# Saltfish-AB/LatentSync

Hardware: AMD Instinct MI355X
Metric: lip-synced frames/sec at 256x256, 16-frame window, 20 DDIM steps (higher is better)
Workload: dtype bf16; 1 GPU; configs[1]: 256x256 x16-frame windows, 20 DDIM steps, guidance 1.0, LatentSync-1.5 UNet + SD-VAE, bf16; 48 independent windows of a clip batched per UNet call; windows_per_rank=240, windows_per_batch=48, frames_per_window=16, global_batch=768, resolution=256, parallelism=dp1 (window sharding, RCCL all-gather of decoded frames)

## Files before the change

### latentsync_amd/csrc/ls_ff.hip

```cpp
#include "ls_common.h"

namespace ls {

struct FFArgs {
  const u16* x;
  const float* ln_mr;
  const u16* w1;
  const float* b1;
  const u16* w2;
  const float* b2;
  u16* y;
  long M;
  int ldx, ldy;
};

template <int C, int I, int PD1 = 2, int PD2 = 6>
__global__ void __launch_bounds__(512, 1) ff_fused_kernel(FFArgs a) {
  constexpr int KT = C / 32;
  constexpr int NCH = I / 32;
  constexpr int WIMG = 64 * (C / 64) * 8;
  constexpr int W2IMG = C * 4;
  constexpr int STAGE = WIMG + W2IMG;
  constexpr int NT2 = C / 16;
  constexpr int PW1 = WIMG / 512;
// ... 107 lines not shown
#pragma unroll
    for (int t = 0; t < NT2; ++t) {
      const int col = 16 * t + 4 * lg;
      const float4 b = *(const float4*)(a.b2 + col);
      const uint2 rs = *(const uint2*)(xr + col);
      const float o0 = out[t][0] + b.x + __uint_as_float(rs.x << 16);
      const float o1 = out[t][1] + b.y + __uint_as_float(rs.x & 0xffff0000u);
      const float o2 = out[t][2] + b.z + __uint_as_float(rs.y << 16);
      const float o3 = out[t][3] + b.w + __uint_as_float(rs.y & 0xffff0000u);
      *(uint2*)(yr + col) = make_uint2(pack2(o0, o1), pack2(o2, o3));
    }
  }
}

struct FFChainArgs {
  const u16* o;
  const u16* wo;
  const float* bo;
  const u16* h1;
  const u16* w1;
  const float* b1;
  const u16* w2;
  const float* b2;
  const u16* wp;
  const float* bp;
  const u16* xb;
  u16* z;
  float* cs_out;
  long M;
  int ldo, ldh, ldxb, ldz;
  float eps;
};

template <int C, int I>
__global__ void __launch_bounds__(512, 1) ff_chain_kernel(FFChainArgs a) {
  constexpr int FMR = 1;
  constexpr int NW = 8 / FMR;
  constexpr int NT = 64 * NW;
  constexpr int KT = C / 32;
  constexpr int NCH = I / 32;
  constexpr int WIMG = 64 * (C / 64) * 8;
  constexpr int W2IMG = C * 4;
  constexpr int STAGE = WIMG + W2IMG;
  constexpr int KPS = STAGE / W2IMG;
  constexpr int NA = (KT + KPS - 1) / KPS;
  constexpr int NT2 = C / 16;
  constexpr int PW1 = WIMG / NT;
  constexpr int UW2 = W2IMG / 64;
  constexpr int PD1 = 2, PD2 = 6;
  constexpr int ZP = C + 8;
  constexpr int RG = NT >= C ? 4 : 2;
  static_assert(STAGE % W2IMG == 0 && KPS >= 1 && WIMG % NT == 0, "ff_chain stage layout");
  static_assert(2 * STAGE * 16 >= 128 * ZP * 2 + RG * (C / 4) * 8 * 4, "ff_chain epilogue LDS");
  static_assert(C == 320 && I == 1280, "ff_chain shape");
  extern __shared__ __attribute__((aligned(16))) uint4 lds[];
  float* b1s = (float*)(lds + 2 * STAGE);

  const int tid = threadIdx.x, lane = tid & 63, wid = tid >> 6;
  const int l16 = lane & 15, lg = lane >> 4;
  const long row0 = (long)blockIdx.x * 128;
  const int wr0 = wid * 16 * FMR + l16;

  for (int i = tid; i < 2 * I / 4; i += NT) ((float4*)b1s)[i] = ((const float4*)a.b1)[i];

  const int wid_u = __builtin_amdgcn_readfirstlane(wid);
  __builtin_assume(wid_u >= 0 && wid_u < NW);
  const i32x4 rs_w1 = buffer_rsrc(a.w1, (uint32_t)(2L * I * C * 2));
  const i32x4 rs_w2 = buffer_rsrc(a.w2, (uint32_t)((long)I * C * 2));
  const i32x4 rs_wo = buffer_rsrc(a.wo, (uint32_t)((long)C * C * 2));
  const i32x4 rs_wp = buffer_rsrc(a.wp, (uint32_t)((long)C * C * 2));
  int vo1[PW1];
#pragma unroll
  for (int p = 0; p < PW1; ++p) {
    const int q = p * NT + tid, r = (q >> 3) & 63, pc = q & 7;
    const int lc = pc ^ ((r >> 1) & 7);
    vo1[p] = (r * C + (q >> 9) * 64 + lc * 8) * 2;
  }
  const int vol = (wid_u * 64 + lane) * 16;
  lds_u4* const lbase = (lds_u4*)lds;
  auto issue = [&](int g, int st) __attribute__((always_inline)) {
    lds_u4* const dst = lbase + st * STAGE;
    if (g < NA || g >= NA + NCH) {
      const bool o = g < NA;
      const int q = o ? g : g - NA - NCH;
      const int nk = min(KPS, KT - q * KPS);
      const int so = q * KPS * W2IMG * 16;
      for (int k = 0; wid_u + k * NW < nk * UW2; ++k)
        ls_raw_buffer_load_lds(o ? rs_wo : rs_wp, (__attribute__((address_space(3))) void*)(dst + (wid_u + k * NW) * 64),
                               16, vol + k * NW * 1024, so, 0, 0);
    } else {
      const int c = g - NA;
#pragma unroll
      for (int p = 0; p < PW1; ++p)
        ls_raw_buffer_load_lds(rs_w1, (__attribute__((address_space(3))) void*)(dst + p * NT + wid_u * 64), 16, vo1[p],
                               c * 64 * C * 2, 0, 0);
      for (int k = 0; wid_u + k * NW < UW2; ++k)
        ls_raw_buffer_load_lds(rs_w2, (__attribute__((address_space(3))) void*)(dst + WIMG + (wid_u + k * NW) * 64), 16,
                               vol + k * NW * 1024, c * W2IMG * 16, 0, 0);
    }
  };
  auto top = [&](int g) __attribute__((always_inline)) {
    wait_vm<0>();
    asm volatile("s_waitcnt lgkmcnt(0)" ::: "memory");
    __builtin_amdgcn_s_barrier();
    asm volatile("" ::: "memory");
    if (g + 1 < 2 * NA + NCH) issue(g + 1, (g + 1) & 1);
    return (const uint4*)(lds + (g & 1) * STAGE);
  };
  issue(0, 0);

  const int p2 = lg ^ (((l16 >> 3) & 1) << 1);
  bf16x8 ar[FMR][KT];
  f32x4 out[FMR][NT2];
  auto init_cols = [&](const float* v) __attribute__((always_inline)) {
#pragma unroll
    for (int t = 0; t < NT2; ++t) {
      const float4 b = *(const float4*)(v + 16 * t + 4 * lg);
#pragma unroll
      for (int f = 0; f < FMR; ++f) out[f][t] = (f32x4){b.x, b.y, b.z, b.w};
    }
  };
  auto proj = [&](int g0) __attribute__((always_inline)) {
#pragma unroll
    for (int q = 0; q < NA; ++q) {
      const uint4* cur = top(g0 + q);
      const int nk = (q + 1) * KPS <= KT ? KPS : KT - q * KPS;
      int lo[KPS];
#pragma unroll
      for (int j = 0; j < KPS; ++j) {
        lo[j] = j * W2IMG + l16 * 4 + p2;
        asm volatile("" : "+v"(lo[j]));
      }
      uint4 wq[PD2];
#pragma unroll
      for (int i = 0; i < PD2; ++i) wq[i] = cur[lo[i / NT2] + (i % NT2) * 64];
#pragma unroll
      for (int j = 0; j < KPS; ++j) {
        if (j < nk) {
          const int k = q * KPS + j < KT ? q * KPS + j : 0;
#pragma unroll
          for (int t = 0; t < NT2; ++t) {
            const int i = j * NT2 + t;
            const bf16x8 wv = __builtin_bit_cast(bf16x8, wq[i % PD2]);
            const int n = i + PD2;
            if (n < nk * NT2) wq[i % PD2] = cur[lo[n / NT2 < KPS ? n / NT2 : 0] + (n % NT2) * 64];
#pragma unroll
            for (int f = 0; f < FMR; ++f)
              out[f][t] = __builtin_amdgcn_mfma_f32_16x16x32_bf16(wv, ar[f][k], out[f][t], 0, 0, 0);
          }
          __builtin_amdgcn_sched_barrier(0);
        }
      }
    }
  };
  auto acc_to_operand = [&](int f, float mean, float rstd) __attribute__((always_inline)) {
#pragma unroll
    for (int s = 0; s < KT; ++s) {
      bf16x8 v;
#pragma unroll
      for (int e = 0; e < 8; ++e) v[e] = (__bf16)((out[f][2 * s + (e >> 2)][e & 3] - mean) * rstd);
      ar[f][s] = v;
    }
  };

#pragma unroll
  for (int f = 0; f < FMR; ++f) {
    const u16* src = a.o + (row0 + wr0 + 16 * f) * a.ldo + lg * 8;
#pragma unroll
    for (int s = 0; s < KT; ++s) ar[f][s] = *(const bf16x8*)(src + s * 32);
  }
  init_cols(a.bo);
  proj(0);
#pragma unroll
  for (int f = 0; f < FMR; ++f) {
    uint2 xr[NT2];
    const u16* hr = a.h1 + (row0 + wr0 + 16 * f) * a.ldh + 4 * lg;
#pragma unroll
    for (int t = 0; t < NT2; ++t) xr[t] = *(const uint2*)(hr + 16 * t);
    float s1 = 0.f;
#pragma unroll
    for (int t = 0; t < NT2; ++t) {
      const uint2 rs = xr[t];
      const uint32_t pk0 = pack2(out[f][t][0] + __uint_as_float(rs.x << 16), out[f][t][1] + __uint_as_float(rs.x & 0xffff0000u));
      const uint32_t pk1 = pack2(out[f][t][2] + __uint_as_float(rs.y << 16), out[f][t][3] + __uint_as_float(rs.y & 0xffff0000u));
      out[f][t] = (f32x4){__uint_as_float(pk0 << 16), __uint_as_float(pk0 & 0xffff0000u),
                          __uint_as_float(pk1 << 16), __uint_as_float(pk1 & 0xffff0000u)};
      s1 += (out[f][t][0] + out[f][t][1]) + (out[f][t][2] + out[f][t][3]);
    }
    const float mean = xor16_32_sum(s1) * (1.0f / C);
    float s2 = 0.f;
#pragma unroll
    for (int t = 0; t < NT2; ++t)
#pragma unroll
      for (int r = 0; r < 4; ++r) {
        const float d = out[f][t][r] - mean;
        s2 = fmaf(d, d, s2);
      }
    const float rstd = rsqrtf(xor16_32_sum(s2) * (1.0f / C) + a.eps);
    acc_to_operand(f, mean, rstd);
  }
#pragma unroll
  for (int t = 0; t < NT2; ++t) {
    const float4 b = *(const float4*)(a.b2 + 16 * t + 4 * lg);
#pragma unroll
    for (int f = 0; f < FMR; ++f) {
      out[f][t][0] += b.x; out[f][t][1] += b.y; out[f][t][2] += b.z; out[f][t][3] += b.w;
    }
  }

  for (int c = 0; c < NCH; ++c) {
    const uint4* cur = top(NA + c);
    f32x4 acc[FMR][4];
    const float* bb = b1s + c * 64 + 4 * lg;
#pragma unroll
    for (int f = 0; f < FMR; ++f)
#pragma unroll
      for (int t = 0; t < 4; ++t) acc[f][t] = (f32x4){0.f, 0.f, 0.f, 0.f};
    auto frag = [&](int s, int t) {
      return __builtin_bit_cast(bf16x8, cur[(s >> 1) * 512 + swz64(t * 16 + l16, (s & 1) * 4 + lg)]);
    };
    const uint4* w2 = cur + WIMG;
    bf16x8 wf[PD1][4];
#pragma unroll
    for (int p = 0; p < PD1; ++p)
#pragma unroll
      for (int t = 0; t < 4; ++t) wf[p][t] = frag(p, t);
    uint4 w2q[PD2];
#pragma unroll
    for (int s = 0; s < KT; ++s) {
      const int sl = s % PD1;
      bf16x8 cw[4];
#pragma unroll
      for (int t = 0; t < 4; ++t) cw[t] = wf[sl][t];
      if (s + PD1 < KT) {
#pragma unroll
        for (int t = 0; t < 4; ++t) wf[sl][t] = frag(s + PD1, t);
      } else if (s + PD1 - KT < PD2) {
        w2q[s + PD1 - KT] = w2[((s + PD1 - KT) * 16 + l16) * 4 + p2];
      }
#pragma unroll
      for (int t = 0; t < 4; ++t)
#pragma unroll
        for (int f = 0; f < FMR; ++f) acc[f][t] = __builtin_amdgcn_mfma_f32_16x16x32_bf16(cw[t], ar[f][s], acc[f][t], 0, 0, 0);
    }
#pragma unroll
    for (int q = PD1; q < PD2; ++q) w2q[q] = w2[(q * 16 + l16) * 4 + p2];
    bf16x8 gv[FMR];
#pragma unroll
    for (int f = 0; f < FMR; ++f)
#pragma unroll
      for (int r = 0; r < 4; ++r) {
        gv[f][r] = (__bf16)((acc[f][0][r] + bb[r]) * gelu_erf(acc[f][1][r] + bb[16 + r]));
        gv[f][4 + r] = (__bf16)((acc[f][2][r] + bb[32 + r]) * gelu_erf(acc[f][3][r] + bb[48 + r]));
      }
#pragma unroll
    for (int t = 0; t < NT2; ++t) {
      const bf16x8 wv = __builtin_bit_cast(bf16x8, w2q[t % PD2]);
      if (t + PD2 < NT2) w2q[t % PD2] = w2[((t + PD2) * 16 + l16) * 4 + p2];
#pragma unroll
      for (int f = 0; f < FMR; ++f) out[f][t] = __builtin_amdgcn_mfma_f32_16x16x32_bf16(wv, gv[f], out[f][t], 0, 0, 0);
    }
  }

#pragma unroll
  for (int f = 0; f < FMR; ++f) acc_to_operand(f, 0.f, 1.f);
  init_cols(a.bp);
  proj(NA + NCH);

  __syncthreads();
  u16* zimg = (u16*)lds;
#pragma unroll
  for (int f = 0; f < FMR; ++f) {
    uint2 xr[NT2];
    const u16* src = a.xb + (row0 + wr0 + 16 * f) * a.ldxb + 4 * lg;
#pragma unroll
    for (int t = 0; t < NT2; ++t) xr[t] = *(const uint2*)(src + 16 * t);
#pragma unroll
    for (int t = 0; t < NT2; ++t) {
      const uint2 rs = xr[t];
      const float o0 = out[f][t][0] + __uint_as_float(rs.x << 16), o1 = out[f][t][1] + __uint_as_float(rs.x & 0xffff0000u);
      const float o2 = out[f][t][2] + __uint_as_float(rs.y << 16), o3 = out[f][t][3] + __uint_as_float(rs.y & 0xffff0000u);
      *(uint2*)(zimg + (wr0 + 16 * f) * ZP + 16 * t + 4 * lg) = make_uint2(pack2(o0, o1), pack2(o2, o3));
    }
  }
  __syncthreads();
  constexpr int PCS = C / 8;
  for (int q = tid; q < 128 * PCS; q += NT) {
    const int r = q / PCS, ch = q - r * PCS;
    *(uint4*)(a.z + (row0 + r) * a.ldz + ch * 8) = *(const uint4*)(zimg + r * ZP + ch * 8);
  }
  if (a.cs_out) {
    constexpr int RPG = 128 / RG;
    float* part = (float*)(zimg + 128 * ZP);
    if (tid < RG * (C / 4)) {
      const int cq = tid % (C / 4), rg = tid / (C / 4);
      float s1[4] = {0.f, 0.f, 0.f, 0.f}, s2[4] = {0.f, 0.f, 0.f, 0.f};
      for (int r = 0; r < RPG; ++r) {
        const uint2 v = *(const uint2*)(zimg + (RPG * rg + r) * ZP + 4 * cq);
        const float fv[4] = {__uint_as_float(v.x << 16), __uint_as_float(v.x & 0xffff0000u),
                             __uint_as_float(v.y << 16), __uint_as_float(v.y & 0xffff0000u)};
// ... 14 lines not shown
        t2 += part[(rg * (C / 4) + cq) * 8 + 4 + e];
      }
      a.cs_out[(long)blockIdx.x * 2 * C + col] = t1;
      a.cs_out[(long)blockIdx.x * 2 * C + C + col] = t2;
    }
  }
}


}

using namespace ls;

extern "C" int ls_ff_chain(const ls_ff_chain_desc* d, void* stream) {
  if (!d || !d->o || !d->wo || !d->bo || !d->h1 || !d->w1 || !d->b1 || !d->w2 || !d->b2 || !d->wp || !d->bp ||
      !d->xb || !d->z)
    return fail(LS_ERR_INVALID, "ls_ff_chain: null pointer");
  if (d->C != 320 || d->inner != 1280) return fail(LS_ERR_INVALID, "ls_ff_chain: C = 320, inner = 1280 only");
  if (d->M <= 0 || d->M % 128 || (d->M / 128) > 0x7fffffffL)
    return fail(LS_ERR_INVALID, "ls_ff_chain: M a positive multiple of 128");
  if (d->ldo < d->C || d->ldh < d->C || d->ldxb < d->C || d->ldz < d->C || d->ldo % 8 || d->ldh % 4 ||
      d->ldxb % 4 || d->ldz % 8)
    return fail(LS_ERR_INVALID, "ls_ff_chain: pitches >= C (o, z: % 8; h1, xb: % 4)");
  if ((((uintptr_t)d->o | (uintptr_t)d->wo | (uintptr_t)d->w1 | (uintptr_t)d->w2 | (uintptr_t)d->wp |
        (uintptr_t)d->b1 | (uintptr_t)d->b2 | (uintptr_t)d->bo | (uintptr_t)d->bp | (uintptr_t)d->z |
        (uintptr_t)d->cs_out) & 15) || (((uintptr_t)d->h1 | (uintptr_t)d->xb) & 7))
    return fail(LS_ERR_INVALID, "ls_ff_chain: operands 16-B aligned (h1 / xb 8-B)");
  FFChainArgs a;
  a.o = (const u16*)d->o; a.wo = (const u16*)d->wo; a.bo = d->bo; a.h1 = (const u16*)d->h1;
  a.w1 = (const u16*)d->w1; a.b1 = d->b1; a.w2 = (const u16*)d->w2; a.b2 = d->b2;
  a.wp = (const u16*)d->wp; a.bp = d->bp; a.xb = (const u16*)d->xb; a.z = (u16*)d->z; a.cs_out = d->cs_out;
  a.M = d->M; a.ldo = d->ldo; a.ldh = d->ldh; a.ldxb = d->ldxb; a.ldz = d->ldz; a.eps = d->eps;
  constexpr int C = 320, I = 1280;
  const size_t shm = (size_t)2 * (64 * (C / 64) * 8 + C * 4) * 16 + 2 * I * sizeof(float);
  LS_SET_MAX_DYN_SHM((ff_chain_kernel<C, I>), (int)shm);
  ff_chain_kernel<C, I><<<(unsigned)(d->M / 128), 512, shm, (hipStream_t)stream>>>(a);
  return check_launch("ff_chain_kernel");
}

extern "C" int ls_feedforward(const ls_ff_desc* d, void* stream) {
  if (!d || !d->x || !d->ln_rowstats || !d->w1 || !d->b1 || !d->w2 || !d->b2 || !d->y)
    return fail(LS_ERR_INVALID, "ls_feedforward: null pointer");
  if (d->C != 320 || d->inner != 1280) return fail(LS_ERR_INVALID, "ls_feedforward: C = 320, inner = 1280 only");
  if (d->M <= 0 || d->ldx < d->C || d->ldy < d->C || d->ldx % 8 || d->ldy % 4)
    return fail(LS_ERR_INVALID, "ls_feedforward: bad rows / pitches (ldx % 8, ldy % 4, >= C)");
  if ((((uintptr_t)d->x | (uintptr_t)d->w1 | (uintptr_t)d->w2 | (uintptr_t)d->b1 | (uintptr_t)d->b2) & 15) ||
      (((uintptr_t)d->y | (uintptr_t)d->ln_rowstats) & 7))
    return fail(LS_ERR_INVALID, "ls_feedforward: x / w1 / w2 / b1 / b2 16-B aligned, y / ln_rowstats 8-B aligned");
  if ((d->M + 127) / 128 > 0x7fffffffL) return fail(LS_ERR_INVALID, "ls_feedforward: too many rows");
  FFArgs a;
  a.x = (const u16*)d->x; a.ln_mr = d->ln_rowstats; a.w1 = (const u16*)d->w1; a.b1 = d->b1;
  a.w2 = (const u16*)d->w2; a.b2 = d->b2; a.y = (u16*)d->y; a.M = d->M; a.ldx = d->ldx; a.ldy = d->ldy;
  constexpr int C = 320, I = 1280;
  const size_t shm = (size_t)2 * (64 * (C / 64) * 8 + C * 4) * 16 + 2 * I * sizeof(float);
  LS_SET_MAX_DYN_SHM((ff_fused_kernel<C, I>), (int)shm);
  ff_fused_kernel<C, I><<<(unsigned)((d->M + 127) / 128), 512, shm, (hipStream_t)stream>>>(a);
  return check_launch("ff_fused_kernel");
}
```

### latentsync_amd/ops.py

```python
import ctypes as C
import math

import torch

from . import _lib
from ._lib import check

ACT_NONE, ACT_GEGLU, ACT_GELU, ACT_SILU = 0, 1, 2, 3
_GN_EPILOGUE = True
GN_SLOT_ROWS = 128
_UPS_PHASE = True


def _p(t):
    return None if t is None else t.data_ptr()


def _stream():
    return torch.cuda.current_stream().cuda_stream


class Workspace:

    def __init__(self, device, gemm_bytes=256 << 20, gn_bytes=24 << 20):
# ... 278 lines not shown


def feedforward(x2d, ln_stats, w1: "Packed", w2: "Packed", w2ff, out=None):
    lib = _lib.load()
    M, C_ = x2d.shape
    if out is None:
        out = torch.empty((M, C_), dtype=torch.bfloat16, device=x2d.device)
    d = _lib.FFDesc()
    d.x, d.ln_rowstats, d.w1, d.b1 = _p(x2d), _p(ln_stats), _p(w1.w), _p(w1.bias)
    d.w2, d.b2, d.y = _p(w2ff), _p(w2.bias), _p(out)
    d.M, d.ldx, d.ldy, d.C, d.inner = M, x2d.stride(0), out.stride(0), C_, w1.N // 2
    check(lib.ls_feedforward(C.byref(d), _stream()), "ls_feedforward")
    return out


class FFChainPack:

    def __init__(self, wo, bo, w1, b1, w2, b2, wp, bp, C, inner, eps):
        self.wo, self.bo, self.w1, self.b1, self.w2, self.b2, self.wp, self.bp = wo, bo, w1, b1, w2, b2, wp, bp
        self.C, self.inner, self.eps = C, inner, eps


def pack_ff_chain(wo: "Packed", ff1: "Packed", ff2: "Packed", po: "Packed", eps=1e-5):
    from .packing import pack_ff_w2, permute_k_acc
    Cc = wo.N
    bf = lambda t: t.to(torch.bfloat16).contiguous()
    w1 = permute_k_acc(ff1.w.float())
    return FFChainPack(bf(pack_ff_w2(wo.w.float()[:, :Cc], permute=False)), wo.bias.float().contiguous(), bf(w1),
                       ff1.bias.float().contiguous(), bf(pack_ff_w2(ff2.w.float()[:, :ff2.K])),
                       ff2.bias.float().contiguous(), bf(pack_ff_w2(po.w.float()[:, :Cc])),
                       po.bias.float().contiguous(), Cc, ff1.N // 2, eps)


def ff_chain_ok(o2d, pk: "FFChainPack"):
    return (pk is not None and o2d.shape[1] == 320 and pk.inner == 1280 and o2d.shape[0] % 128 == 0
            and o2d.stride(1) == 1 and o2d.stride(0) % 8 == 0)


def ff_chain(o2d, h1, xb, pk: "FFChainPack", shape=None, gn_out=True):
    lib = _lib.load()
    M, C_ = o2d.shape
    res = torch.empty(shape or (M, C_), dtype=torch.bfloat16, device=o2d.device)
    out = res.view(M, C_)
    cs = torch.empty((M // GN_SLOT_ROWS, 2, C_), dtype=torch.float32, device=o2d.device) if gn_out else None
    d = _lib.FFChainDesc()
    d.o, d.wo, d.bo, d.h1 = _p(o2d), _p(pk.wo), _p(pk.bo), _p(h1)
    d.w1, d.b1, d.w2, d.b2, d.wp, d.bp = _p(pk.w1), _p(pk.b1), _p(pk.w2), _p(pk.b2), _p(pk.wp), _p(pk.bp)
    d.xb, d.z, d.cs_out = _p(xb), _p(out), _p(cs)
    d.M, d.ldo, d.ldh, d.ldxb, d.ldz = M, o2d.stride(0), h1.stride(0), xb.stride(0), out.stride(0)
    d.C, d.inner, d.eps = C_, pk.inner, float(pk.eps)
    check(lib.ls_ff_chain(C.byref(d), _stream()), "ls_ff_chain")
    if cs is not None:
        res.gn_cs = cs
    return res


class XAttnPack:

    def __init__(self, wq, bq, wo, bo, C, heads):
        self.wq, self.bq, self.wo, self.bo, self.C, self.heads = wq, bq, wo, bo, C, heads


def pack_cross_attention(wq, ln_weight, ln_bias, wo, bo, heads, device):
    from .packing import pack_xattn_q, pack_xattn_wo
    w = wq.float().cpu()
    gamma, beta = ln_weight.float().cpu(), ln_bias.float().cpu()
    pq, pb = pack_xattn_q(w * gamma[None, :], w @ beta, heads)
    po = pack_xattn_wo(wo.float().cpu(), heads)
    bf = lambda t: t.to(torch.bfloat16).to(device).contiguous()
# ... 442 lines not shown
```

### latentsync_amd/unet.py

```python
import math
from dataclasses import dataclass

import torch

from . import ops
from .config import STAGE2_MODEL
from .packing import geglu_interleave, pack_ff_w2, pack_phase_weight, pack_weight, pad_bias
from .schema import unet_param_shapes
from .weights import fill_state_dict

_FUSED_TEMPORAL = True
_FUSED_FF = True
_FF_CHAIN = True
_NARROW_OUT = True
_FUSED_XATTN = False


def _ff(h, st, ff1, ff2, ff2p):
    if ff2p is not None and ops.feedforward_ok(h, ff1, ff2):
        return ops.feedforward(h, st, ff1, ff2, ff2p)
    g = ops.linear(h, ff1, act=ops.ACT_GEGLU, ln_stats=st)
    return ops.linear(g, ff2, res=h)


# ... 139 lines not shown
        self.chain = _chain_pack(self.o2, self.ff1, self.ff2, self.proj_out, c) if self.has_audio else None

    def audio_kv(self, audio_rows):
        return ops.linear(audio_rows, self.kv2) if self.has_audio else None

    def __call__(self, x, audio_rows, n_audio_tok, kv=None):
        n, H, W, C = x.shape
        HW = H * W
        rows = n * HW
        d = C // self.heads
        sc = ops.group_norm(x, self.groups, 1e-6, *self.norm, n)
        st = torch.empty((rows, 2), dtype=torch.float32, device=x.device)
        h = ops.conv(x, self.proj_in, aff=(sc[0], sc[1], 1, False), aff_materialize=True,
                     stats_out=st).view(rows, C)
        qkv = ops.linear(h, self.qkv1, ln_stats=st)
        o = torch.empty((rows, C), dtype=torch.bfloat16, device=x.device)
        ops.attention(qkv, qkv[:, C:], qkv[:, 2 * C:], o, batch=n, z2=1, heads=self.heads, nq=HW, nk=HW, head_dim=d,
                      qs=(HW * 3 * C, 0, 3 * C, d), ks=(HW * 3 * C, 0, 3 * C, d), vs=(HW * 3 * C, 0, 3 * C, d),
                      os_=(HW * C, 0, C, d), fp8=self.fp8 and HW > 128 and d in (40, 80))
        h = ops.linear(o, self.o1, res=h, stats_out=st)
        if self.has_audio and audio_rows is not None:
            if kv is None:
                kv = ops.linear(audio_rows, self.kv2)
            L = n_audio_tok
            if ops.cross_attention_ok(h, self.xa, L, HW):
                st2 = torch.empty_like(st)
                h = ops.cross_attention_block(h, st, self.xa, kv, L, HW, st2)
                st = st2
                return self._tail(x, h, st, n, H, W, C)
            q = ops.linear(h, self.q2, ln_stats=st)
            ops.attention(q, kv, kv[:, C:], o, batch=n, z2=1, heads=self.heads, nq=HW, nk=L, head_dim=d,
                          qs=(HW * C, 0, C, d), ks=(L * 2 * C, 0, 2 * C, d), vs=(L * 2 * C, 0, 2 * C, d),
                          os_=(HW * C, 0, C, d))
            if ops.ff_chain_ok(o, self.chain):
                return ops.ff_chain(o, h, x.view(rows, C), self.chain, shape=(n, H, W, C))
            h = ops.linear(o, self.o2, res=h, stats_out=st)
        return self._tail(x, h, st, n, H, W, C)

    def _tail(self, x, h, st, n, H, W, C):
        h = _ff(h, st, self.ff1, self.ff2, self.ff2p)
        return ops.conv(h.view(n, H, W, C), self.proj_out, res=x, gn_out=True)


class _Motion:
    def __init__(self, dv, p, c, heads, groups, kw):
        t = p + ".temporal_transformer"
        b = t + ".transformer_blocks.0"
        sd = dv.sd
        self.c, self.heads, self.groups = c, heads, groups
        self.norm = (dv.f32(t + ".norm.weight"), dv.f32(t + ".norm.bias"))
        self.proj_in = dv.packed(t + ".proj_in.weight", t + ".proj_in.bias")
        self.proj_out = dv.packed(t + ".proj_out.weight", t + ".proj_out.bias")
        self.attn = []
        i = 0
        max_len = kw.get("temporal_position_encoding_max_len", 24)
        while f"{b}.attention_blocks.{i}.to_q.weight" in sd:
            a = f"{b}.attention_blocks.{i}"
            pe = sd.get(a + ".pos_encoder.pe")
            if kw.get("temporal_position_encoding", False):
                pe = (pe.reshape(-1, c) if pe is not None else positional_encoding(c, max_len)).float()
                pe = pe.to(dv.device).contiguous()
            else:
                pe = None
            ln = (sd[f"{b}.norms.{i}.weight"], sd[f"{b}.norms.{i}.bias"])
            wqkv = [sd[f"{a}.to_{n}.weight"] for n in "qkv"]
            self.attn.append(dict(
                qkv=dv.packed_ln(torch.cat(wqkv, 0), None, ln, pe=pe),
                fused=ops.pack_temporal(*wqkv, *ln, pe, heads, dv.device) if c in (320, 640) and heads == 8
                else None,
                o=dv.packed(a + ".to_out.0.weight", a + ".to_out.0.bias")))
            i += 1
        self.ff1 = dv.packed_ln(sd[b + ".ff.net.0.proj.weight"], sd[b + ".ff.net.0.proj.bias"],
                                (sd[b + ".ff_norm.weight"], sd[b + ".ff_norm.bias"]), geglu=True)
        self.ff2 = dv.packed(b + ".ff.net.2.weight", b + ".ff.net.2.bias")
        self.ff2p = _ff2_packed(dv, b + ".ff.net.2.weight")
        self.chain = _chain_pack(self.attn[-1]["o"], self.ff1, self.ff2, self.proj_out, c) if self.attn else None

    def __call__(self, x, B):
        n, H, W, C = x.shape
        F = n // B
        S = H * W
        rows = n * S
        d = C // self.heads
        sc = ops.group_norm(x, self.groups, 1e-6, *self.norm, n)
        lns = torch.empty((rows, 2), dtype=torch.float32, device=x.device)
        h = ops.conv(x, self.proj_in, aff=(sc[0], sc[1], 1, False), aff_materialize=True,
                     stats_out=lns).view(rows, C)
        o = torch.empty((rows, C), dtype=torch.bfloat16, device=x.device)
        fuse = _FUSED_TEMPORAL and ops.temporal_attention_ok(C, self.heads, F, S)
        for i, a in enumerate(self.attn):
            if fuse and a["fused"] is not None:
                ops.temporal_attention(h, a["fused"], B, F, S, out=o)
            else:
                pk = a["qkv"]
                rv = (pk.pe_rows, S, pk.pe_rows.shape[1], F) if pk.pe_rows is not None else None
                qkv = ops.linear(h, pk, ln_stats=lns, rowvec=rv)
                st = (F * S * 3 * C, 3 * C, S * 3 * C, d)
                ops.attention(qkv, qkv[:, C:], qkv[:, 2 * C:], o, batch=B * S, z2=S, heads=self.heads, nq=F, nk=F,
                              head_dim=d, qs=st, ks=st, vs=st, os_=(F * S * C, C, S * C, d))
            if i == len(self.attn) - 1 and ops.ff_chain_ok(o, self.chain):
                return ops.ff_chain(o, h, x.view(rows, C), self.chain, shape=(n, H, W, C))
            h = ops.linear(o, a["o"], res=h, stats_out=lns)
        h = _ff(h, lns, self.ff1, self.ff2, self.ff2p)
        return ops.conv(h.view(n, H, W, C), self.proj_out, res=x, gn_out=True)


class _DeviceUNet:

    def __init__(self, sd, cfg, device):
        dv = _Dev(sd, device)
        self.cfg, self.device = cfg, device
        boc = list(cfg["block_out_channels"])
        nb = len(boc)
        heads = cfg["attention_head_dim"]
        heads = list(heads) if isinstance(heads, (list, tuple)) else [heads] * nb
        groups, eps = cfg["norm_num_groups"], float(cfg["norm_eps"])
        lpb = cfg["layers_per_block"]
        audio = cfg["add_audio_layer"]
        mkw = cfg.get("motion_module_kwargs") or {}
        mheads = mkw.get("num_attention_heads", 8)
        self.cin = cfg["in_channels"]
        self.cin_pad = (self.cin + 7) // 8 * 8
        self.cout = cfg["out_channels"]
        self.boc = boc
        self.temb_dim = boc[0] * 4
        self.flip, self.shift = bool(cfg["flip_sin_to_cos"]), float(cfg["freq_shift"])
        bfw = lambda k: sd[k].to(torch.bfloat16).to(device).contiguous()
        self.t1, self.t1b = bfw("time_embedding.linear_1.weight"), dv.f32("time_embedding.linear_1.bias")
        self.t2, self.t2b = bfw("time_embedding.linear_2.weight"), dv.f32("time_embedding.linear_2.bias")
        self.conv_in = dv.packed("conv_in.weight", "conv_in.bias", cin_pad=self.cin_pad)
        temb_w, temb_b = [], []

        def resnet(p, cin, cout, scale=1.0):
# ... 328 lines not shown
```

### latentsync_amd/csrc/ls_conv_halo.hip

```cpp
#include "ls_conv.h"

namespace ls {

template <int TW, int BN, int TH_ = 256 / TW>
struct HaloCfg {
  static constexpr int TH = TH_;
  static constexpr int WNW = BN >= 64 ? 2 : 1;
  static constexpr int NT = (TH / 4) * WNW * 64;
  static constexpr bool COMPACT = TH < 16;
  static constexpr int P = COMPACT ? TW + 2 : TW + 8;
  static constexpr int HALO = (TH + 2) * P * 8;
  static constexpr int WSLOT = BN * 8;
  static constexpr int NSW = COMPACT ? 2 : BN <= 128 ? 3 : 2;
  static constexpr int DPT = (WSLOT + NT - 1) / NT;
  static constexpr int FN = BN / WNW / 16;
  static constexpr size_t SHM = ((size_t)2 * HALO + (size_t)NSW * WSLOT + 64 + 64) * 16;
  static_assert(SHM <= (COMPACT ? 81920 : 163840), "halo conv LDS (compact: two blocks per CU)");
  static_assert((size_t)64 * (BN + 4) * 4 <= (size_t)2 * HALO * 16, "epilogue staging fits the halo images");
  static_assert(TW == 16 && (TH == 16 || TH == 8), "16-pixel patch rows, 16 or 8 of them");
  static_assert(BN % (16 * WNW) == 0, "whole 16-column fragments per wave");
  static constexpr int MINB = BN >= 64 ? 16 / TH : 2;
};


// ... 141 lines not shown
      const bool live = WSLOT % NT == 0 || j * NT + wid_u * 64 < WSLOT;
      ls_raw_buffer_load_lds(rs_w, (__attribute__((address_space(3))) void*)(live ? slot + j * NT : dummy_l), 16, wvo[j],
                             g * 128, 0, 0);
    }
  };

  static_assert(TW == 16, "fragment i = one patch row");
  const int p0 = 64 * wm + l16;
  const int hp0 = (p0 / TW) * P + (p0 % TW) + (COMPACT ? 0 : 3) + py * P + px;

  f32x4 acc[FM][FN];
#pragma unroll
  for (int i = 0; i < FM; ++i)
#pragma unroll
    for (int j = 0; j < FN; ++j) acc[i][j] = (f32x4){0.f, 0.f, 0.f, 0.f};

  for (int g = 0; g < NSW - 1 && g < G; ++g) issue_w(g, g % NSW);
  {
    uint4 hpre[NHL];
    if constexpr (GN) load_par(0);
#pragma unroll
    for (int j = 0; j < NHL; ++j) {
      const int vo = hpix[j] >= 0 ? hpix[j] * a.ld1 * 2 + hc8 * 16 : (int)0x80000000;
      hpre[j] = __builtin_bit_cast(uint4, ls_raw_buffer_load_v4(rs1, vo, 0, 0));
    }
    if constexpr (GN) {
      store_par(0);
      __syncthreads();
    }
    put_halo(0, 0, NHL, hpre);
  }

  bf16x8 apf[2][FM];
  auto read_a = [&](const uint4* hb, int tt) {
    constexpr int TPR = PH ? 2 : 3;
    const int hpt = hp0 + (tt / TPR) * P + tt % TPR;
    const int sw = COMPACT ? (l16 + px + tt % TPR) & 7 : hpt & 7;
#pragma unroll
    for (int ks = 0; ks < 2; ++ks) {
      const int base = hpt * 8 + ((ks * 4 + lg) ^ sw);
#pragma unroll
      for (int i = 0; i < FM; ++i)
        apf[ks][i] = __builtin_bit_cast(bf16x8, hb[base + 8 * (((16 * i) / TW) * P + (16 * i) % TW)]);
    }
  };
  auto tap = [&](int ci, int par, auto t_tag, auto last_tag) {
    constexpr int t = decltype(t_tag)::value;
    constexpr bool LAST = decltype(last_tag)::value;
    const int g = NTAP * ci + t;
    const int hpar = ci & 1;
    constexpr int HY = LAST ? 0 : (t - 1 >= 0 ? halo_issue(t - 1, NHL, GN, TS) : 0) +
                                  (NSW >= 3 && t - 2 >= 0 ? halo_issue(t - 2, NHL, GN, TS) : 0);
    if (g + NSW - 2 >= G) wait_vm<0>();
    else wait_vm<(NSW - 2) * DPT + HY>();
    asm volatile("s_waitcnt lgkmcnt(0)" ::: "memory");
    __builtin_amdgcn_s_barrier();
    asm volatile("" ::: "memory");
    if (g + NSW - 1 < G) issue_w(g + NSW - 1, wslot(par, t + NSW - 1));
    if constexpr (!LAST) {
      if constexpr (GN && t == 1) store_par(ci + 1);
      if constexpr (t == TS || t == 2 * TS) store_halo(hpar ^ 1, t / TS - 1);
      if constexpr (t == 0 || t == TS || t == 2 * TS) load_halo(ci + 1, t / TS);
    }
    const uint4* hb = hbuf + hpar * HALO;
    const uint4* wb = wbuf + wslot(par, t) * WSLOT;
    if constexpr (t == 0) read_a(hb, 0);
#pragma unroll
    for (int ks = 0; ks < 2; ++ks) {
      bf16x8 bfr[FN];
#pragma unroll
      for (int j = 0; j < FN; ++j)
        bfr[j] = __builtin_bit_cast(bf16x8, wb[swz64(wn * WTN + j * 16 + l16, ks * 4 + lg)]);
#pragma unroll
      for (int i = 0; i < FM; ++i)
#pragma unroll
        for (int j = 0; j < FN; ++j)
          acc[i][j] = __builtin_amdgcn_mfma_f32_16x16x32_bf16(apf[ks][i], bfr[j], acc[i][j], 0, 0, 0);
    }
    if constexpr (t < NTAP - 1) read_a(hb, t + 1);
    if constexpr (!LAST && t == NTAP - 1) store_halo(hpar ^ 1, 2);
  };
  using I0 = std::integral_constant<int, 0>; using I1 = std::integral_constant<int, 1>;
  using I2 = std::integral_constant<int, 2>; using I3 = std::integral_constant<int, 3>;
  using I4 = std::integral_constant<int, 4>; using I5 = std::integral_constant<int, 5>;
  using I6 = std::integral_constant<int, 6>; using I7 = std::integral_constant<int, 7>;
  using I8 = std::integral_constant<int, 8>;
  auto chunk = [&](int ci, auto last) {
    const int par = PH && NSW == 3 ? ci % 3 : ci & 1;
    tap(ci, par, I0{}, last); tap(ci, par, I1{}, last); tap(ci, par, I2{}, last);
    tap(ci, par, I3{}, last);
    if constexpr (!PH) {
      tap(ci, par, I4{}, last); tap(ci, par, I5{}, last);
      tap(ci, par, I6{}, last); tap(ci, par, I7{}, last); tap(ci, par, I8{}, last);
    }
  };
  for (int ci = 0; ci + 1 < nchunk; ++ci) chunk(ci, std::false_type{});
  chunk(nchunk - 1, std::true_type{});
  asm volatile("s_waitcnt lgkmcnt(0)" ::: "memory");
  __builtin_amdgcn_s_barrier();
  asm volatile("" ::: "memory");
  const int m0v = PH ? (int)(img * 4 * HW) + ((ph * tpc + tyb) * tpr + txb) * (TH * TW)
                     : (int)(img * HW) + (tyb * tpr + txb) * (TH * TW);
  const long m0r = PH ? img * 4 * HW + (long)(2 * y0 + py) * a.Wo + 2 * x0 + px : img * HW + (long)y0 * a.W + x0;
  static_assert((size_t)(NT / (BN / 8)) * BN * 2 * 4 <= (size_t)2 * HALO * 16, "column-sum partials fit the halo images");
  store_tile_plain<TH * TW, BN, TH / 4, WNW, false, CSF, PH ? -TW : TW, 2>(a, acc, (float*)lds_dyn, m0v, n0, m0r);
}

bool halo_ok(const ls_conv_desc* d, const ConvArgs& a) {
  if (!g_tune.halo || g_tune.force_tile || g_tune.force_regstage || d->ksize != 3 || a.stride != 1 || a.pad != 1 ||
      !a.ccm || a.Cin % 64 || a.C1 % 64 || a.K != (a.upsample == 2 ? 4 : 9) * a.Cin || a.y_f32 || a.act != LS_ACT_NONE ||
      a.ln_mr || a.stats_out || a.ldy % 8 || (a.res && a.ldr % 8))
    return false;
  if (a.upsample ? (!g_tune.halo_ups || a.aff_scale || a.Ho != 2 * a.H || a.Wo != 2 * a.W) : (a.Ho != a.H || a.Wo != a.W))
// ... 67 lines not shown
```

Before: 156.9 frames/s.

## Warp-specialize ff_chain FF loop with ping-pong halves and separate W1/W2 rings

Restructures the ff_chain kernel's feed-forward loop so that the two halves of the workgroup's waves alternate between compute and loading. One half loads W1 chunks and the other loads W2 images into separate rings (2 W1 slots, 3 W2 slots). Each segment fuses the W2 down-projection of the previous chunk with the W1 up-projection of the current one. It adds s_setprio hints and sched_group_barrier interleaving to overlap LDS reads with MFMA work. The LDS footprint grows, and the Python guard is tightened to check the residual tensors' strides and alignment.

```diff
diff --git a/latentsync_amd/csrc/ls_ff.hip b/latentsync_amd/csrc/ls_ff.hip
--- a/latentsync_amd/csrc/ls_ff.hip
+++ b/latentsync_amd/csrc/ls_ff.hip
@@ -163,6 +163,23 @@
   float eps;
 };
 
+constexpr int ff_chain_ring_u4(int C) { return 2 * (64 * (C / 64) * 8) + 3 * (C * 4); }
+
+__device__ __forceinline__ void dma16(const i32x4& rs, lds_u4* dst, int voff, int soff) {
+  unsigned keep;
+  asm volatile("s_mov_b32 %0, m0\n\ts_mov_b32 m0, %1\n\ts_nop 0\n\tbuffer_load_dwordx4 %2, %3, %4 offen lds\n\ts_mov_b32 m0, %0"
+               : "=&s"(keep)
+               : "s"((unsigned)(size_t)dst), "v"(voff), "s"(rs), "s"(soff)
+               : "memory");
+}
+
+#ifndef LS_FFC_QD
+#define LS_FFC_QD 8
+#endif
+#ifndef LS_FFC_PRIO
+#define LS_FFC_PRIO 1
+#endif
+
 template <int C, int I>
 __global__ void __launch_bounds__(512, 1) ff_chain_kernel(FFChainArgs a) {
   constexpr int FMR = 1;
@@ -175,17 +192,25 @@
   constexpr int STAGE = WIMG + W2IMG;
   constexpr int KPS = STAGE / W2IMG;
   constexpr int NA = (KT + KPS - 1) / KPS;
+  constexpr int NW1 = 2, NW2 = 3;
+  constexpr int W2R = NW1 * WIMG;
+  constexpr int RING = ff_chain_ring_u4(C);
   constexpr int NT2 = C / 16;
-  constexpr int PW1 = WIMG / NT;
+  constexpr int PW1 = WIMG / 256;
   constexpr int UW2 = W2IMG / 64;
-  constexpr int PD1 = 2, PD2 = 6;
+  constexpr int PD2 = 6;
+  constexpr int QD = LS_FFC_QD;
   constexpr int ZP = C + 8;
   constexpr int RG = NT >= C ? 4 : 2;
-  static_assert(STAGE % W2IMG == 0 && KPS >= 1 && WIMG % NT == 0, "ff_chain stage layout");
-  static_assert(2 * STAGE * 16 >= 128 * ZP * 2 + RG * (C / 4) * 8 * 4, "ff_chain epilogue LDS");
+  static_assert(FMR == 1 && STAGE % W2IMG == 0 && KPS >= 1 && WIMG % 256 == 0 && UW2 % 4 == 0, "ff_chain stage layout");
+  static_assert(RING == W2R + NW2 * W2IMG && RING >= 2 * STAGE, "ff_chain rings cover the two stages");
+  static_assert(RING * 16 + 2 * I * 4 <= 163840, "ff_chain LDS");
+  static_assert(RING * 16 >= 128 * ZP * 2 + RG * (C / 4) * 8 * 4, "ff_chain epilogue LDS");
+  static_assert(((NA - 1) & 1) == 1 && WIMG <= STAGE && W2R >= STAGE + (KT - (NA - 1) * KPS) * W2IMG, "ff_chain A -> B");
+  static_assert(NCH % 2 == 0 && NCH >= 4 && WIMG == 2 * W2IMG && KPS == 3, "ff_chain B -> C");
   static_assert(C == 320 && I == 1280, "ff_chain shape");
   extern __shared__ __attribute__((aligned(16))) uint4 lds[];
-  float* b1s = (float*)(lds + 2 * STAGE);
+  float* b1s = (float*)(lds + RING);
 
   const int tid = threadIdx.x, lane = tid & 63, wid = tid >> 6;
   const int l16 = lane & 15, lg = lane >> 4;
@@ -196,49 +221,49 @@
 
   const int wid_u = __builtin_amdgcn_readfirstlane(wid);
   __builtin_assume(wid_u >= 0 && wid_u < NW);
+  const int half = wid_u >> 2, w4 = wid_u & 3;
   const i32x4 rs_w1 = buffer_rsrc(a.w1, (uint32_t)(2L * I * C * 2));
   const i32x4 rs_w2 = buffer_rsrc(a.w2, (uint32_t)((long)I * C * 2));
   const i32x4 rs_wo = buffer_rsrc(a.wo, (uint32_t)((long)C * C * 2));
   const i32x4 rs_wp = buffer_rsrc(a.wp, (uint32_t)((long)C * C * 2));
-  int vo1[PW1];
-#pragma unroll
-  for (int p = 0; p < PW1; ++p) {
-    const int q = p * NT + tid, r = (q >> 3) & 63, pc = q & 7;
-    const int lc = pc ^ ((r >> 1) & 7);
-    vo1[p] = (r * C + (q >> 9) * 64 + lc * 8) * 2;
-  }
+  const int t4 = tid & 255;
+  const int vo1 = ((t4 >> 3) * C + ((t4 & 7) ^ ((t4 >> 4) & 7)) * 8) * 2;
   const int vol = (wid_u * 64 + lane) * 16;
+  const int vol4 = (w4 * 64 + lane) * 16;
   lds_u4* const lbase = (lds_u4*)lds;
-  auto issue = [&](int g, int st) __attribute__((always_inline)) {
+  auto issue_proj = [&](bool o, int q, int st) __attribute__((always_inline)) {
     lds_u4* const dst = lbase + st * STAGE;
-    if (g < NA || g >= NA + NCH) {
-      const bool o = g < NA;
-      const int q = o ? g : g - NA - NCH;
-      const int nk = min(KPS, KT - q * KPS);
-      const int so = q * KPS * W2IMG * 16;
-      for (int k = 0; wid_u + k * NW < nk * UW2; ++k)
-        ls_raw_buffer_load_lds(o ? rs_wo : rs_wp, (__attribute__((address_space(3))) void*)(dst + (wid_u + k * NW) * 64),
-                               16, vol + k * NW * 1024, so, 0, 0);
-    } else {
-      const int c = g - NA;
-#pragma unroll
-      for (int p = 0; p < PW1; ++p)
-        ls_raw_buffer_load_lds(rs_w1, (__attribute__((address_space(3))) void*)(dst + p * NT + wid_u * 64), 16, vo1[p],
-                               c * 64 * C * 2, 0, 0);
-      for (int k = 0; wid_u + k * NW < UW2; ++k)
-        ls_raw_buffer_load_lds(rs_w2, (__attribute__((address_space(3))) void*)(dst + WIMG + (wid_u + k * NW) * 64), 16,
-                               vol + k * NW * 1024, c * W2IMG * 16, 0, 0);
-    }
-  };
-  auto top = [&](int g) __attribute__((always_inline)) {
+    const int nk = min(KPS, KT - q * KPS);
+    const int so = q * KPS * W2IMG * 16;
+    for (int k = 0; wid_u + k * NW < nk * UW2; ++k)
+      ls_raw_buffer_load_lds(o ? rs_wo : rs_wp, (__attribute__((address_space(3))) void*)(dst + (wid_u + k * NW) * 64),
+                             16, vol + k * NW * 1024, so, 0, 0);
+  };
+  auto issue_w1 = [&](int c) __attribute__((always_inline)) {
+    lds_u4* const dst = lbase + (c & (NW1 - 1)) * WIMG + w4 * 64;
+#pragma unroll
+    for (int p = 0; p < PW1; ++p)
+      dma16(rs_w1, dst + p * 256, vo1, c * 64 * C * 2 + (p & 1) * 32 * C * 2 + (p >> 1) * 128);
+  };
+  auto issue_img = [&](const i32x4& rs, int img, int dst_u4) __attribute__((always_inline)) {
+    lds_u4* const dst = lbase + dst_u4 + w4 * 64;
+#pragma unroll
+    for (int k = 0; k < UW2 / 4; ++k)
+      dma16(rs, dst + k * 256, vol4, img * W2IMG * 16 + k * 4096);
+  };
+  auto top = [&](bool o, int q) __attribute__((always_inline)) {
     wait_vm<0>();
     asm volatile("s_waitcnt lgkmcnt(0)" ::: "memory");
     __builtin_amdgcn_s_barrier();
     asm volatile("" ::: "memory");
-    if (g + 1 < 2 * NA + NCH) issue(g + 1, (g + 1) & 1);
-    return (const uint4*)(lds + (g & 1) * STAGE);
-  };
-  issue(0, 0);
+    if (q + 1 < NA) issue_proj(o, q + 1, (q + 1) & 1);
+    else if (o) {
+      if (half) issue_w1(0);
+      else issue_img(rs_w2, 0, W2R);
+    }
+    return (const uint4*)(lds + (q & 1) * STAGE);
+  };
+  issue_proj(true, 0, 0);
 
   const int p2 = lg ^ (((l16 >> 3) & 1) << 1);
   bf16x8 ar[FMR][KT];
@@ -251,10 +276,10 @@
       for (int f = 0; f < FMR; ++f) out[f][t] = (f32x4){b.x, b.y, b.z, b.w};
     }
   };
-  auto proj = [&](int g0) __attribute__((always_inline)) {
+  auto proj = [&](bool o) __attribute__((always_inline)) {
 #pragma unroll
     for (int q = 0; q < NA; ++q) {
-      const uint4* cur = top(g0 + q);
+      const uint4* cur = top(o, q);
       const int nk = (q + 1) * KPS <= KT ? KPS : KT - q * KPS;
       int lo[KPS];
 #pragma unroll
@@ -301,7 +326,7 @@
     for (int s = 0; s < KT; ++s) ar[f][s] = *(const bf16x8*)(src + s * 32);
   }
   init_cols(a.bo);
-  proj(0);
+  proj(true);
 #pragma unroll
   for (int f = 0; f < FMR; ++f) {
     uint2 xr[NT2];
@@ -339,64 +364,91 @@
     }
   }
 
-  for (int c = 0; c < NCH; ++c) {
-    const uint4* cur = top(NA + c);
-    f32x4 acc[FMR][4];
-    const float* bb = b1s + c * 64 + 4 * lg;
-#pragma unroll
-    for (int f = 0; f < FMR; ++f)
-#pragma unroll
-      for (int t = 0; t < 4; ++t) acc[f][t] = (f32x4){0.f, 0.f, 0.f, 0.f};
-    auto frag = [&](int s, int t) {
-      return __builtin_bit_cast(bf16x8, cur[(s >> 1) * 512 + swz64(t * 16 + l16, (s & 1) * 4 + lg)]);
+  f32x4 acc[4];
+  bf16x8 gv = __builtin_bit_cast(bf16x8, make_uint4(0, 0, 0, 0));
+#pragma unroll
+  for (int t = 0; t < 4; ++t) acc[t] = (f32x4){0.f, 0.f, 0.f, 0.f};
+  auto seg_m = [&](int c) __attribute__((always_inline)) {
+    const uint4* w1 = lds + (c & (NW1 - 1)) * WIMG;
+    const uint4* w2 = lds + W2R + (c > 0 ? (unsigned)(c - 1) % NW2 : 0u) * W2IMG;
+    auto frag = [&](int i) {
+      if (i < NT2) return w2[(i * 16 + l16) * 4 + p2];
+      const int s = (i - NT2) >> 2, t = (i - NT2) & 3;
+      return w1[(s >> 1) * 512 + swz64(t * 16 + l16, (s & 1) * 4 + lg)];
     };
-    const uint4* w2 = cur + WIMG;
-    bf16x8 wf[PD1][4];
-#pragma unroll
-    for (int p = 0; p < PD1; ++p)
-#pragma unroll
-      for (int t = 0; t < 4; ++t) wf[p][t] = frag(p, t);
-    uint4 w2q[PD2];
-#pragma unroll
-    for (int s = 0; s < KT; ++s) {
-      const int sl = s % PD1;
-      bf16x8 cw[4];
-#pragma unroll
-      for (int t = 0; t < 4; ++t) cw[t] = wf[sl][t];
-      if (s + PD1 < KT) {
-#pragma unroll
-        for (int t = 0; t < 4; ++t) wf[sl][t] = frag(s + PD1, t);
-      } else if (s + PD1 - KT < PD2) {
-        w2q[s + PD1 - KT] = w2[((s + PD1 - KT) * 16 + l16) * 4 + p2];
-      }
-#pragma unroll
-      for (int t = 0; t < 4; ++t)
-#pragma unroll
-        for (int f = 0; f < FMR; ++f) acc[f][t] = __builtin_amdgcn_mfma_f32_16x16x32_bf16(cw[t], ar[f][s], acc[f][t], 0, 0, 0);
-    }
-#pragma unroll
-    for (int q = PD1; q < PD2; ++q) w2q[q] = w2[(q * 16 + l16) * 4 + p2];
-    bf16x8 gv[FMR];
-#pragma unroll
-    for (int f = 0; f < FMR; ++f)
-#pragma unroll
-      for (int r = 0; r < 4; ++r) {
-        gv[f][r] = (__bf16)((acc[f][0][r] + bb[r]) * gelu_erf(acc[f][1][r] + bb[16 + r]));
-        gv[f][4 + r] = (__bf16)((acc[f][2][r] + bb[32 + r]) * gelu_erf(acc[f][3][r] + bb[48 + r]));
-      }
-#pragma unroll
-    for (int t = 0; t < NT2; ++t) {
-      const bf16x8 wv = __builtin_bit_cast(bf16x8, w2q[t % PD2]);
-      if (t + PD2 < NT2) w2q[t % PD2] = w2[((t + PD2) * 16 + l16) * 4 + p2];
-#pragma unroll
-      for (int f = 0; f < FMR; ++f) out[f][t] = __builtin_amdgcn_mfma_f32_16x16x32_bf16(wv, gv[f], out[f][t], 0, 0, 0);
-    }
-  }
+    constexpr int NM = NT2 + 4 * KT;
+    uint4 q[QD];
+#pragma unroll
+    for (int i = 0; i < QD; ++i) q[i] = frag(i);
+#pragma unroll
+    for (int i = 0; i < NM; ++i) {
+      const bf16x8 f = __builtin_bit_cast(bf16x8, q[i % QD]);
+      if (i + QD < NM) q[i % QD] = frag(i + QD);
+      if (i < NT2) {
+        out[0][i] = __builtin_amdgcn_mfma_f32_16x16x32_bf16(f, gv, out[0][i], 0, 0, 0);
+      } else {
+        const int s = (i - NT2) >> 2, t = (i - NT2) & 3;
+        acc[t] = __builtin_amdgcn_mfma_f32_16x16x32_bf16(f, ar[0][s], s ? acc[t] : (f32x4){0.f, 0.f, 0.f, 0.f}, 0, 0, 0);
+      }
+    }
+    __builtin_amdgcn_sched_group_barrier(0x100, QD, 0);
+#pragma unroll
+    for (int i = 0; i < NM - QD; ++i) {
+      __builtin_amdgcn_sched_group_barrier(0x008, 1, 0);
+      __builtin_amdgcn_sched_group_barrier(0x100, 1, 0);
+    }
+    __builtin_amdgcn_sched_group_barrier(0x008, QD, 0);
+  };
+#if LS_FFC_PRIO == 2
+  if (half) __builtin_amdgcn_s_setprio(1);
+#endif
+  wait_vm<0>();
+  asm volatile("s_waitcnt lgkmcnt(0)" ::: "memory");
+  for (int hp = 0; hp < 2 * NCH + 2; ++hp) {
+    __builtin_amdgcn_s_barrier();
+    asm volatile("" ::: "memory");
+    const int c = (hp - half) >> 1;
+    if (((hp + half) & 1) == 0) {
+#if LS_FFC_PRIO == 1
+      __builtin_amdgcn_s_setprio(1);
+#endif
+      seg_m(c);
+#if LS_FFC_PRIO == 1
+      __builtin_amdgcn_s_setprio(0);
+#endif
+      asm volatile("s_waitcnt lgkmcnt(0)" ::: "memory");
+      if (half) wait_vm<0>();
+    } else {
+      if (half) {
+        if (c + 2 < NCH) issue_w1(c + 2);
+        else if (c + 2 == NCH) { issue_img(rs_wp, 0, 0); issue_img(rs_wp, 1, W2IMG); }
+        else issue_img(rs_wp, 2, 2 * W2IMG);
+      } else if (c + 1 < NCH) {
+        issue_img(rs_w2, c + 1, W2R + ((unsigned)(c + 1) % NW2) * W2IMG);
+      }
+      if (c >= 0 && c < NCH) {
+        const float* bb = b1s + c * 64 + 4 * lg;
+#pragma unroll
+        for (int r = 0; r < 4; ++r) {
+          gv[r] = (__bf16)((acc[0][r] + bb[r]) * gelu_erf(acc[1][r] + bb[16 + r]));
+          gv[4 + r] = (__bf16)((acc[2][r] + bb[32 + r]) * gelu_erf(acc[3][r] + bb[48 + r]));
+        }
+      }
+      asm volatile("s_waitcnt lgkmcnt(0)" ::: "memory");
+      if (!half) {
+        if (c + 1 < NCH) wait_vm<UW2 / 4>();
+        else wait_vm<0>();
+      }
+    }
+  }
+#if LS_FFC_PRIO == 2
+  if (half) __builtin_amdgcn_s_setprio(0);
+#endif
 
 #pragma unroll
   for (int f = 0; f < FMR; ++f) acc_to_operand(f, 0.f, 1.f);
   init_cols(a.bp);
-  proj(NA + NCH);
+  proj(false);
 
   __syncthreads();
   u16* zimg = (u16*)lds;
@@ -477,7 +529,7 @@
   a.wp = (const u16*)d->wp; a.bp = d->bp; a.xb = (const u16*)d->xb; a.z = (u16*)d->z; a.cs_out = d->cs_out;
   a.M = d->M; a.ldo = d->ldo; a.ldh = d->ldh; a.ldxb = d->ldxb; a.ldz = d->ldz; a.eps = d->eps;
   constexpr int C = 320, I = 1280;
-  const size_t shm = (size_t)2 * (64 * (C / 64) * 8 + C * 4) * 16 + 2 * I * sizeof(float);
+  const size_t shm = (size_t)ff_chain_ring_u4(C) * 16 + 2 * I * sizeof(float);
   LS_SET_MAX_DYN_SHM((ff_chain_kernel<C, I>), (int)shm);
   ff_chain_kernel<C, I><<<(unsigned)(d->M / 128), 512, shm, (hipStream_t)stream>>>(a);
   return check_launch("ff_chain_kernel");
diff --git a/latentsync_amd/ops.py b/latentsync_amd/ops.py
--- a/latentsync_amd/ops.py
+++ b/latentsync_amd/ops.py
@@ -334,9 +334,13 @@
                        po.bias.float().contiguous(), Cc, ff1.N // 2, eps)
 
 
-def ff_chain_ok(o2d, pk: "FFChainPack"):
-    return (pk is not None and o2d.shape[1] == 320 and pk.inner == 1280 and o2d.shape[0] % 128 == 0
-            and o2d.stride(1) == 1 and o2d.stride(0) % 8 == 0)
+def ff_chain_ok(o2d, pk: "FFChainPack", h1=None, xb=None):
+    def rows(t, pitch, align):
+        return (t.dim() == 2 and t.shape == o2d.shape and t.stride(1) == 1 and t.stride(0) >= t.shape[1]
+                and t.stride(0) % pitch == 0 and t.data_ptr() % align == 0)
+    return (pk is not None and o2d.dim() == 2 and o2d.shape[1] == 320 and pk.inner == 1280
+            and o2d.shape[0] > 0 and o2d.shape[0] % 128 == 0 and rows(o2d, 8, 16)
+            and all(rows(t, 4, 8) for t in (h1, xb) if t is not None))
 
 
 def ff_chain(o2d, h1, xb, pk: "FFChainPack", shape=None, gn_out=True):
diff --git a/latentsync_amd/unet.py b/latentsync_amd/unet.py
--- a/latentsync_amd/unet.py
+++ b/latentsync_amd/unet.py
@@ -195,7 +195,7 @@
             ops.attention(q, kv, kv[:, C:], o, batch=n, z2=1, heads=self.heads, nq=HW, nk=L, head_dim=d,
                           qs=(HW * C, 0, C, d), ks=(L * 2 * C, 0, 2 * C, d), vs=(L * 2 * C, 0, 2 * C, d),
                           os_=(HW * C, 0, C, d))
-            if ops.ff_chain_ok(o, self.chain):
+            if ops.ff_chain_ok(o, self.chain, h, x.view(rows, C)):
                 return ops.ff_chain(o, h, x.view(rows, C), self.chain, shape=(n, H, W, C))
             h = ops.linear(o, self.o2, res=h, stats_out=st)
         return self._tail(x, h, st, n, H, W, C)
@@ -261,7 +261,7 @@
                 st = (F * S * 3 * C, 3 * C, S * 3 * C, d)
                 ops.attention(qkv, qkv[:, C:], qkv[:, 2 * C:], o, batch=B * S, z2=S, heads=self.heads, nq=F, nk=F,
                               head_dim=d, qs=st, ks=st, vs=st, os_=(F * S * C, C, S * C, d))
-            if i == len(self.attn) - 1 and ops.ff_chain_ok(o, self.chain):
+            if i == len(self.attn) - 1 and ops.ff_chain_ok(o, self.chain, h, x.view(rows, C)):
                 return ops.ff_chain(o, h, x.view(rows, C), self.chain, shape=(n, H, W, C))
             h = ops.linear(o, a["o"], res=h, stats_out=lns)
         h = _ff(h, lns, self.ff1, self.ff2, self.ff2p)
```

Result: no change. 157.5 frames/s, median of 6 (+0.4%).

## Interleave LDS fragment reads with MFMAs and relax lgkmcnt wait in halo conv

Applied to the files above, without the earlier changes.

Splits the A-fragment prefetch and B-fragment reads of each conv tap into per-k-slice pieces and interleaves them with MFMA groups, using sched_barrier to pin the order. The weight issue and halo load/store traffic move after the first B read, and the per-tap lgkmcnt wait now leaves FM outstanding LDS reads in flight instead of draining to zero. The aim is to hide LDS latency behind matrix math in the implicit-GEMM conv. In exchange it relies on careful counter accounting: if the outstanding-count assumption is wrong, reads could race. The fixed scheduling may also add register pressure.

```diff
diff --git a/latentsync_amd/csrc/ls_conv_halo.hip b/latentsync_amd/csrc/ls_conv_halo.hip
--- a/latentsync_amd/csrc/ls_conv_halo.hip
+++ b/latentsync_amd/csrc/ls_conv_halo.hip
@@ -197,17 +197,14 @@
   }
 
   bf16x8 apf[2][FM];
-  auto read_a = [&](const uint4* hb, int tt) {
+  auto read_a = [&](const uint4* hb, int tt, int ks) {
     constexpr int TPR = PH ? 2 : 3;
     const int hpt = hp0 + (tt / TPR) * P + tt % TPR;
     const int sw = COMPACT ? (l16 + px + tt % TPR) & 7 : hpt & 7;
-#pragma unroll
-    for (int ks = 0; ks < 2; ++ks) {
-      const int base = hpt * 8 + ((ks * 4 + lg) ^ sw);
-#pragma unroll
-      for (int i = 0; i < FM; ++i)
-        apf[ks][i] = __builtin_bit_cast(bf16x8, hb[base + 8 * (((16 * i) / TW) * P + (16 * i) % TW)]);
-    }
+    const int base = hpt * 8 + ((ks * 4 + lg) ^ sw);
+#pragma unroll
+    for (int i = 0; i < FM; ++i)
+      apf[ks][i] = __builtin_bit_cast(bf16x8, hb[base + 8 * (((16 * i) / TW) * P + (16 * i) % TW)]);
   };
   auto tap = [&](int ci, int par, auto t_tag, auto last_tag) {
     constexpr int t = decltype(t_tag)::value;
@@ -218,32 +215,56 @@
                                   (NSW >= 3 && t - 2 >= 0 ? halo_issue(t - 2, NHL, GN, TS) : 0);
     if (g + NSW - 2 >= G) wait_vm<0>();
     else wait_vm<(NSW - 2) * DPT + HY>();
-    asm volatile("s_waitcnt lgkmcnt(0)" ::: "memory");
+    asm volatile("s_waitcnt lgkmcnt(%0)" ::"n"(t > 0 ? FM : 0) : "memory");
     __builtin_amdgcn_s_barrier();
     asm volatile("" ::: "memory");
-    if (g + NSW - 1 < G) issue_w(g + NSW - 1, wslot(par, t + NSW - 1));
-    if constexpr (!LAST) {
-      if constexpr (GN && t == 1) store_par(ci + 1);
-      if constexpr (t == TS || t == 2 * TS) store_halo(hpar ^ 1, t / TS - 1);
-      if constexpr (t == 0 || t == TS || t == 2 * TS) load_halo(ci + 1, t / TS);
-    }
     const uint4* hb = hbuf + hpar * HALO;
     const uint4* wb = wbuf + wslot(par, t) * WSLOT;
-    if constexpr (t == 0) read_a(hb, 0);
-#pragma unroll
-    for (int ks = 0; ks < 2; ++ks) {
-      bf16x8 bfr[FN];
+    if constexpr (t == 0) {
+      read_a(hb, 0, 0);
+      read_a(hb, 0, 1);
+    }
+    auto read_b = [&](bf16x8* bfr, int ks) {
 #pragma unroll
       for (int j = 0; j < FN; ++j)
         bfr[j] = __builtin_bit_cast(bf16x8, wb[swz64(wn * WTN + j * 16 + l16, ks * 4 + lg)]);
-#pragma unroll
-      for (int i = 0; i < FM; ++i)
+    };
+    auto mfmas = [&](const bf16x8* bfr, int ks, int i0, int i1) {
+#pragma unroll
+      for (int i = i0; i < i1; ++i)
 #pragma unroll
         for (int j = 0; j < FN; ++j)
           acc[i][j] = __builtin_amdgcn_mfma_f32_16x16x32_bf16(apf[ks][i], bfr[j], acc[i][j], 0, 0, 0);
-    }
-    if constexpr (t < NTAP - 1) read_a(hb, t + 1);
-    if constexpr (!LAST && t == NTAP - 1) store_halo(hpar ^ 1, 2);
+    };
+    {
+      bf16x8 bfr0[FN], bfr1[FN];
+      read_b(bfr0, 0);
+      __builtin_amdgcn_sched_barrier(0);
+      if (g + NSW - 1 < G) issue_w(g + NSW - 1, wslot(par, t + NSW - 1));
+      if constexpr (!LAST) {
+        if constexpr (GN && t == 1) store_par(ci + 1);
+        if constexpr (t == 0) load_halo(ci + 1, 0);
+      }
+      __builtin_amdgcn_sched_barrier(0);
+      mfmas(bfr0, 0, 0, FM - 1);
+      read_b(bfr1, 1);
+      mfmas(bfr0, 0, FM - 1, FM);
+      if constexpr (t < NTAP - 1) {
+        __builtin_amdgcn_sched_barrier(0);
+        read_a(hb, t + 1, 0);
+      }
+      mfmas(bfr1, 1, 0, FM);
+    }
+    if constexpr (!LAST && (t == TS || t == 2 * TS || t == NTAP - 1)) {
+      __builtin_amdgcn_sched_barrier(0);
+      store_halo(hpar ^ 1, t == NTAP - 1 ? 2 : t / TS - 1);
+      if constexpr (t < NTAP - 1) load_halo(ci + 1, t / TS);
+    }
+    if constexpr (t < NTAP - 1) {
+      __builtin_amdgcn_sched_barrier(0);
+      read_a(hb, t + 1, 1);
+      __builtin_amdgcn_sched_barrier(0);
+    }
   };
   using I0 = std::integral_constant<int, 0>; using I1 = std::integral_constant<int, 1>;
   using I2 = std::integral_constant<int, 2>; using I3 = std::integral_constant<int, 3>;
```

Result: faster. 154.8 frames/s before, 156.5 frames/s after (median of 6 runs) (+1.1%).
